# leaner-forever/SEGS-SLAM

Hardware: AMD Instinct MI355X
Metric: mapper train-iters/sec (fwd+bwd raster) (higher is better)
Workload: dtype f32; 1 GPU; 1080p_3m: 3000000 Gaussians, 1920x1080, 1 keyframe per GPU, fwd+bwd raster; P=3000000, P_visible=2096178, num_rendered=10472370, instances_binned=7913347, instances_live=6766534, width=1920, height=1080, parallelism=keyframe-dp1, forward=resident (no host sync), hipgraph=off

## Files before the change

segs-slam_amd/csrc/binning.hip:

```cpp
#include <hip/hip_runtime.h>
#include <cstdint>
#include "gs_layout.h"
#include "kernels.h"

namespace segs {

constexpr int PREFIX_ROWS = PREFIX_ROWS_PER_WG;

__global__ void __launch_bounds__(1024) scan_block_sums_kernel(uint32_t* __restrict__ block_sums, int nblocks,
                                                               const uint32_t* __restrict__ depth_range,
                                                               uint32_t* __restrict__ total) {
  __shared__ uint32_t w_sum[16], w_dmax[16], w_dnmin[16];
  const int tid = threadIdx.x, lane = tid & 63, wv = tid >> 6;
  uint32_t sum = 0, dmax = 0, dnmin = 0;
  for (int i = tid; i < nblocks; i += 1024) {
    sum += block_sums[i];
    dmax = max(dmax, depth_range[i]);
    dnmin = max(dnmin, depth_range[nblocks + i]);
  }
#pragma unroll
  for (int off = 32; off > 0; off >>= 1) {
    sum += __shfl_down(sum, off, 64);
    dmax = max(dmax, (uint32_t)__shfl_down((int)dmax, off, 64));
    dnmin = max(dnmin, (uint32_t)__shfl_down((int)dnmin, off, 64));
// ... 200 lines not shown
  const uint64_t kc = km.dbits < 0 ? (key >> 32) : (((key >> 32) << km.dbits) | (uint64_t)((uint32_t)key - km.dmin));
  return (uint32_t)(kc >> shift) & ((1u << BITS) - 1u);
}
template <int BITS>
__device__ __forceinline__ uint32_t digit_of(uint32_t key, int shift, KeyMap km) { return ((key - km.dmin) >> shift) & ((1u << BITS) - 1u); }

template <int BITS>
__device__ __forceinline__ uint64_t match_digit(uint32_t d, uint64_t valid, int nbits) {
  uint64_t peers = valid;
#pragma unroll
  for (int bit = 0; bit < BITS; bit++) {
    if (bit < nbits) {
      const bool set = (d >> bit) & 1u;
      const uint64_t m = __ballot(set);
      peers &= set ? m : ~m;
    }
  }
  return peers;
}
__device__ __forceinline__ uint32_t mbcnt(uint64_t m) {
  return __builtin_amdgcn_mbcnt_hi((uint32_t)(m >> 32), __builtin_amdgcn_mbcnt_lo((uint32_t)m, 0u));
}

template <typename K, int BITS>
__global__ void __launch_bounds__(SORT_THREADS) radix_count_kernel(const K* __restrict__ keys, int n, int shift,
                                                                    uint32_t dmin, int dbits,
                                                                    uint32_t* __restrict__ tile_prefix, uint32_t* __restrict__ chunk_hist,
                                                                    int nblocks, int nchunks,
                                                                    const uint32_t* __restrict__ n_dev, int drop_dead, int chunk_tiles,
                                                                    int nbits ) {
  const KeyMap km{dmin, dbits};
  if (n_dev) n = (int)min(*n_dev, (uint32_t)n);
  constexpr int NDIG = 1 << BITS;
  constexpr int DPT = NDIG / SORT_THREADS;
  __shared__ uint32_t cnt[4][NDIG];
  const int tid = threadIdx.x, lane = tid & 63, wv = tid >> 6;
  const uint32_t dmask = (1u << nbits) - 1u;
  uint32_t* my = cnt[wv];
  uint32_t running[DPT];
#pragma unroll
  for (int j = 0; j < DPT; j++) running[j] = 0u;
  K kreg[SORT_ITEMS_PER_THREAD], knext[SORT_ITEMS_PER_THREAD];
  const int chunks_in_use = (int)(((size_t)n + (size_t)SORT_TILE * chunk_tiles - 1) / ((size_t)SORT_TILE * chunk_tiles));
  const int chunks_per_xcd = (chunks_in_use + 7) >> 3;
  const int chunk_id = (int)(blockIdx.x & 7u) * chunks_per_xcd + (int)(blockIdx.x >> 3);
  if ((int)(blockIdx.x >> 3) >= chunks_per_xcd) {
    const int col = 8 * chunks_per_xcd + ((int)(blockIdx.x >> 3) - chunks_per_xcd) * 8 + (int)(blockIdx.x & 7u);
    if (col < nchunks) {
      constexpr int ND = 1 << BITS;
      for (int d = threadIdx.x; d < ND; d += SORT_THREADS) chunk_hist[(size_t)d * nchunks + col] = 0u;
    }
    return;
  }
  if (chunk_id >= nchunks) return;
  const int b0 = chunk_id * chunk_tiles;
  auto load_tile = [&](int b, K* dst) {
    const size_t wave_base = (size_t)b * SORT_TILE + (size_t)wv * (SORT_TILE / 4);
#pragma unroll
    for (int r = 0; r < SORT_ITEMS_PER_THREAD; r++) {
      const size_t i = wave_base + (size_t)r * 64 + lane;
      dst[r] = (b < nblocks && i < (size_t)n) ? keys[i] : (K)DEAD_KEY_OF(K);
    }
  };
  load_tile(b0, kreg);
  for (int t = 0; t < chunk_tiles; t++) {
    const int b = b0 + t;
    if (b >= nblocks) break;
    for (int i = tid; i < 4 * NDIG; i += SORT_THREADS) (&cnt[0][0])[i] = 0;
    if (t + 1 < chunk_tiles) load_tile(b + 1, knext);
    __syncthreads();
    const size_t wave_base = (size_t)b * SORT_TILE + (size_t)wv * (SORT_TILE / 4);
#pragma unroll
    for (int r = 0; r < SORT_ITEMS_PER_THREAD; r++) {
      const size_t i = wave_base + (size_t)r * 64 + lane;
      if (i < (size_t)n && !(drop_dead && kreg[r] == (K)DEAD_KEY_OF(K))) atomicAdd(&my[digit_of<BITS>(kreg[r], shift, km) & dmask], 1u);
    }
    __syncthreads();
#pragma unroll
    for (int j = 0; j < DPT; j++) {
      const int d = tid * DPT + j;
      tile_prefix[(size_t)b * NDIG + d] = running[j];
      running[j] += cnt[0][d] + cnt[1][d] + cnt[2][d] + cnt[3][d];
    }
    __syncthreads();
#pragma unroll
    for (int r = 0; r < SORT_ITEMS_PER_THREAD; r++) kreg[r] = knext[r];
  }
#pragma unroll
  for (int j = 0; j < DPT; j++) chunk_hist[(size_t)(tid * DPT + j) * nchunks + chunk_id] = running[j];
}

__global__ void __launch_bounds__(256) radix_scan_kernel(uint32_t* __restrict__ block_hist, int nblocks,
                                                         uint32_t* __restrict__ digit_totals) {
  constexpr int ITEMS = 8;
  __shared__ uint32_t wave_tot[4];
  const int tid = threadIdx.x, lane = tid & 63, wv = tid >> 6;
  uint32_t* row = block_hist + (size_t)blockIdx.x * nblocks;
  uint32_t carry = 0;
  for (int base = 0; base < nblocks; base += 256 * ITEMS) {
    const int i0 = base + tid * ITEMS;
    uint32_t v[ITEMS], sum = 0;
#pragma unroll
    for (int q = 0; q < ITEMS; q++) { v[q] = (i0 + q < nblocks) ? row[i0 + q] : 0u; sum += v[q]; }
    uint32_t x = sum;
#pragma unroll
    for (int off = 1; off < 64; off <<= 1) {
      const uint32_t y = __shfl_up(x, off, 64);
      if (lane >= off) x += y;
    }
    if (lane == 63) wave_tot[wv] = x;
    __syncthreads();
    uint32_t wbase = 0, total = 0;
#pragma unroll
    for (int w = 0; w < 4; w++) { const uint32_t t = wave_tot[w]; if (w < wv) wbase += t; total += t; }
    uint32_t run = carry + wbase + x - sum;
#pragma unroll
    for (int q = 0; q < ITEMS; q++) { if (i0 + q < nblocks) row[i0 + q] = run; run += v[q]; }
    carry += total;
    __syncthreads();
  }
  if (tid == 0) digit_totals[blockIdx.x] = carry;
}

template <typename K, int BITS, bool AUX>
__global__ void __launch_bounds__(SORT_THREADS) radix_scatter_kernel(
    const K* __restrict__ keys_in, const uint32_t* __restrict__ vals_in, K* __restrict__ keys_out,
    uint32_t* __restrict__ vals_out, int n, int shift, uint32_t dmin, int dbits, const uint32_t* __restrict__ tile_prefix,
    const uint32_t* __restrict__ chunk_prefix , const uint32_t* __restrict__ digit_totals,
    int nblocks, int nchunks, const uint32_t* __restrict__ n_dev, int drop_dead, uint32_t* __restrict__ n_live_out,
    const uint32_t* __restrict__ aux_in, uint32_t* __restrict__ aux_out, int nbits ,
    int chunk_tiles ,
    int pack_shift ,
    uint2* __restrict__ ranges_out ,
    uint32_t* __restrict__ status, uint32_t* __restrict__ status_mirror ,
    int write_keys ) {
  const KeyMap km{dmin, dbits};
  const uint32_t dmask = (1u << nbits) - 1u;
  if (ranges_out != nullptr && status != nullptr && blockIdx.x == 0 && threadIdx.x == 0) {
    const uint32_t ntot = status[0];
    const uint32_t over = (ntot > (uint32_t)n || status[2] != 0u) ? 1u : 0u;
    status[2] = 0u;
    status[3] = over;
    const uint32_t live = min(n_dev ? *n_dev : ntot, min(ntot, (uint32_t)n));
    status[1] = live;
    if (status_mirror) { status_mirror[0] = ntot; status_mirror[1] = live; status_mirror[3] = over; }
  }
  if (n_dev) n = (int)min(*n_dev, (uint32_t)n);
  constexpr int NDIG = 1 << BITS;
  constexpr int DPT = NDIG / SORT_THREADS;
  static_assert(NDIG % SORT_THREADS == 0 && BITS <= 11, "digit | rank << BITS must fit the rank of 2048 keys");
  __shared__ K s_keys[SORT_TILE];
  __shared__ uint32_t s_vals[SORT_TILE];
  __shared__ uint32_t s_aux[AUX ? SORT_TILE : 1];
  __shared__ uint32_t cnt[4][NDIG];
  __shared__ uint32_t local_start[NDIG];
  __shared__ int32_t gdelta[NDIG];
  __shared__ uint32_t scan_tmp[4];
  const int tid = threadIdx.x, lane = tid & 63, wv = tid >> 6;
  for (int i = tid; i < 4 * NDIG; i += SORT_THREADS) (&cnt[0][0])[i] = 0;
  __syncthreads();

#if defined(SEGS_MEASURE) && defined(SORT_TILE_IDENTITY)
  const int tile_id = (int)blockIdx.x;
#else
  const int tiles_in_use = (int)(((size_t)n + SORT_TILE - 1) / SORT_TILE);
  const int tiles_per_xcd = (tiles_in_use + 7) >> 3;
  const int tile_id = (int)(blockIdx.x & 7u) * tiles_per_xcd + (int)(blockIdx.x >> 3);
  if (tiles_in_use == 0 && n_live_out != nullptr && blockIdx.x == 0 && tid == 0) *n_live_out = 0u;
  if ((int)(blockIdx.x >> 3) >= tiles_per_xcd) return;
#endif
  if (tile_id >= nblocks) return;
  const size_t tile_base = (size_t)tile_id * SORT_TILE;
  const size_t wave_base = tile_base + (size_t)wv * (SORT_TILE / 4);
  const int nvalid = (size_t)n > tile_base ? (int)min((size_t)SORT_TILE, (size_t)n - tile_base) : 0;

  K key[SORT_ITEMS_PER_THREAD];
  uint32_t val[SORT_ITEMS_PER_THREAD];
  uint32_t aux[AUX ? SORT_ITEMS_PER_THREAD : 1];
  uint32_t drank[SORT_ITEMS_PER_THREAD];
  volatile uint32_t* my = cnt[wv];
#pragma unroll
  for (int r = 0; r < SORT_ITEMS_PER_THREAD; r++) {
    const size_t i = wave_base + (size_t)r * 64 + lane;
    const bool valid = i < (size_t)n;
    key[r] = valid ? keys_in[i] : (K)0;
    val[r] = vals_in ? (valid ? vals_in[i] : 0u) : (uint32_t)i;
    if (AUX) aux[r] = valid ? aux_in[val[r]] : 0u;
    if (!AUX && pack_shift > 0 && valid) val[r] |= min(aux_in[i], (0xFFFFFFFFu >> pack_shift)) << pack_shift;
  }
#pragma unroll
  for (int r = 0; r < SORT_ITEMS_PER_THREAD; r++) {
    const size_t i = wave_base + (size_t)r * 64 + lane;
    const bool valid = i < (size_t)n && !(drop_dead && key[r] == (K)DEAD_KEY_OF(K));
    const uint32_t d = valid ? (digit_of<BITS>(key[r], shift, km) & dmask) : 0u;
    const uint64_t vmask = __ballot(valid);
    const uint64_t peers = match_digit<BITS>(d, vmask, nbits);
    const uint32_t below = mbcnt(peers);
    uint32_t old = 0;
    if (valid) old = my[d];
    __builtin_amdgcn_wave_barrier();
    if (valid && below == 0) my[d] = old + (uint32_t)__popcll(peers);
    __builtin_amdgcn_wave_barrier();
    drank[r] = valid ? (d | ((old + below) << BITS)) : 0xFFFFFFFFu;
  }
  __syncthreads();

  uint32_t run[DPT], tot[DPT], thread_run = 0, thread_tot = 0;
#pragma unroll
  for (int j = 0; j < DPT; j++) {
    const int d = tid * DPT + j;
    uint32_t r = 0;
#pragma unroll
    for (int w = 0; w < 4; w++) { const uint32_t c = cnt[w][d]; cnt[w][d] = r; r += c; }
    run[j] = r; thread_run += r;
// ... 11 lines not shown
  for (int off = 1; off < 64; off <<= 1) {
    uint32_t y = __shfl_up(tx, off, 64);
    if (lane >= off) tx += y;
  }
  __shared__ uint32_t tot_tmp[4];
  if (lane == 63) tot_tmp[wv] = tx;
  __syncthreads();
  uint32_t lbase = 0, gbase = 0;
  for (int w = 0; w < wv; w++) { lbase += scan_tmp[w]; gbase += tot_tmp[w]; }
  uint32_t lstart = lbase + x - thread_run, gstart = gbase + tx - thread_tot;
#pragma unroll
  for (int j = 0; j < DPT; j++) {
    const int d = tid * DPT + j;
    local_start[d] = lstart;
    gdelta[d] = (int32_t)(gstart + chunk_prefix[(size_t)d * nchunks + tile_id / chunk_tiles] +
                          tile_prefix[(size_t)tile_id * NDIG + d] - lstart);
    lstart += run[j]; gstart += tot[j];
  }
  const int nout = drop_dead ? (int)(scan_tmp[0] + scan_tmp[1] + scan_tmp[2] + scan_tmp[3]) : nvalid;
  if (n_live_out != nullptr && tile_id == 0 && tid == 0) *n_live_out = tot_tmp[0] + tot_tmp[1] + tot_tmp[2] + tot_tmp[3];
  __syncthreads();

#pragma unroll
  for (int r = 0; r < SORT_ITEMS_PER_THREAD; r++) {
    if (drank[r] != 0xFFFFFFFFu) {
      const uint32_t d = drank[r] & (uint32_t)(NDIG - 1);
      const uint32_t pos = local_start[d] + cnt[wv][d] + (drank[r] >> BITS);
      s_keys[pos] = key[r];
      s_vals[pos] = val[r];
      if (AUX) s_aux[pos] = aux[r];
    }
  }
  __syncthreads();
#pragma unroll 4
  for (int r = 0; r < SORT_ITEMS_PER_THREAD; r++) {
    const int lp = r * SORT_THREADS + tid;
    if (lp < nout) {
      const K k = s_keys[lp];
#if defined(SEGS_MEASURE) && defined(ABLATE_SCATTER_LINEAR)
      const size_t gp = tile_base + (size_t)lp + (size_t)(gdelta[digit_of<BITS>(k, shift, km) & dmask] & 0);
#else
      const size_t gp = (size_t)((int64_t)lp + (int64_t)gdelta[digit_of<BITS>(k, shift, km) & dmask]);
#endif
#if defined(SEGS_MEASURE) && defined(ABLATE_SCATTER_NO_STORE)
      if (k == (K)0x12345677 && gp == 77) keys_out[gp] = k;
      continue;
#endif
      if (write_keys) keys_out[gp] = k;
      vals_out[gp] = s_vals[lp];
      if (AUX) aux_out[gp] = s_aux[lp];
      if constexpr (sizeof(K) == 4) {
        if (ranges_out != nullptr) {
          const K prev = lp > 0 ? s_keys[lp - 1] : ~k, next = lp + 1 < nout ? s_keys[lp + 1] : ~k;
          if (k != prev) atomicMin(&ranges_out[k].x, (uint32_t)gp);
          if (k != next) atomicMax(&ranges_out[k].y, (uint32_t)gp + 1u);
        }
      }
    }
  }
}

#define SEGS_INSTANTIATE_RADIX(K, BITS)                                                                                          \
  template __global__ void radix_count_kernel<K, BITS>(const K*, int, int, uint32_t, int, uint32_t*, uint32_t*, int, int,       \
                                                       const uint32_t*, int, int, int);                                                  \
  template __global__ void radix_scatter_kernel<K, BITS, false>(const K*, const uint32_t*, K*, uint32_t*, int, int, uint32_t, int, \
                                                                const uint32_t*, const uint32_t*, const uint32_t*, int, int,        \
                                                                const uint32_t*, int, uint32_t*, const uint32_t*, uint32_t*, int, int, int, \
                                                                uint2*, uint32_t*, uint32_t*, int);
SEGS_INSTANTIATE_RADIX(uint64_t, 8)
SEGS_INSTANTIATE_RADIX(uint32_t, 8)
SEGS_INSTANTIATE_RADIX(uint32_t, 9)
SEGS_INSTANTIATE_RADIX(uint32_t, 11)
#undef SEGS_INSTANTIATE_RADIX
#define SEGS_INSTANTIATE_AUX(BITS)                                                                                                     \
  template __global__ void radix_scatter_kernel<uint32_t, BITS, true>(const uint32_t*, const uint32_t*, uint32_t*, uint32_t*, int, int, \
                                                                      uint32_t, int, const uint32_t*, const uint32_t*, const uint32_t*, \
                                                                      int, int, const uint32_t*, int, uint32_t*, const uint32_t*, uint32_t*, int, int, int, \
                                                                      uint2*, uint32_t*, uint32_t*, int);
SEGS_INSTANTIATE_AUX(8)
SEGS_INSTANTIATE_AUX(9)
#undef SEGS_INSTANTIATE_AUX

__global__ void __launch_bounds__(256) identify_tile_ranges_kernel(int L, const uint32_t* __restrict__ keys,
                                                                   uint2* __restrict__ ranges, const uint32_t* __restrict__ n_dev,
                                                                   uint32_t* __restrict__ status, uint32_t* __restrict__ status_mirror,
                                                                   const uint32_t* __restrict__ n_live ) {
  static_assert(RANGE_KEYS_PER_THREAD == 4, "one uint4 per thread");
  const int idx = blockIdx.x * 256 + threadIdx.x;
  if (n_dev) {
    const uint32_t n = *n_dev;
    if (idx == 0 && status) {
      const uint32_t over = (n > (uint32_t)L || status[2] != 0u) ? 1u : 0u;
      status[2] = 0u;
      status[3] = over;
      const uint32_t live = n_live ? min(*n_live, min(n, (uint32_t)L)) : min(n, (uint32_t)L);
      status[1] = live;
      if (status_mirror) { status_mirror[0] = n; status_mirror[1] = live; status_mirror[3] = over; }
    }
    L = (int)min(n, (uint32_t)L);
  }
  if (n_live) L = (int)min(*n_live, (uint32_t)L);
  const int i0 = idx * RANGE_KEYS_PER_THREAD;
  if (i0 >= L) return;
// ... 132 lines not shown
```

segs-slam_amd/csrc/capi.hip:

```cpp
#include <hip/hip_runtime.h>
#include <cstdio>
#include <cstdlib>
#include <algorithm>
#include <cstring>
#include <string>
#include <vector>
#include "../../include/segs_raster.h"
#include "gs_layout.h"
#include "kernels.h"

using namespace segs;

namespace {
thread_local std::string g_err;
}
int segs::set_error(int code, const char* what) {
  g_err = what;
  return code;
}
int segs::set_hip_error(hipError_t e, const char* where) {
  g_err = std::string(where) + ": " + hipGetErrorString(e);
  return (int)e > 0 ? (int)e : 1;
}

// ... 48 lines not shown
uint32_t getHigherMsb(uint32_t n) {
  uint32_t msb = sizeof(n) * 4, step = msb;
  while (step > 1) {
    step /= 2;
    if (n >> msb) msb += step; else msb -= step;
  }
  if (n >> msb) msb++;
  return msb;
}

int count_chunk_tiles(int nblocks) {
#ifdef SEGS_MEASURE
  static const int chunk_override = [] { const char* e = getenv("SEGS_COUNT_CHUNK"); const int v = e ? atoi(e) : 0; return (v == 1 || v == 2 || v == 4) ? v : 0; }();
  if (chunk_override > 0) return chunk_override;
#endif
  return nblocks <= 256 ? 1 : (nblocks <= 2048 ? 2 : SORT_COUNT_CHUNK_TILES);
}
struct SortFusion {
  uint2* ranges = nullptr;
  uint32_t* status = nullptr;
  uint32_t* status_mirror = nullptr;
  bool keep_sorted_keys = true;
};
template <typename K, int BITS = 8>
int sort_pairs(char* bin, const BinningLayout& L, int n, int end_bit, uint32_t dmin, int dbits, hipStream_t st,
               const uint32_t* n_dev = nullptr, bool drop_dead = false, bool iota_vals = false, const uint32_t* aux_in = nullptr,
               uint32_t* aux_final = nullptr, int pack_shift = 0 ,
               const SortFusion& fuse = SortFusion(), const K* first_keys = nullptr ) {
  if (n <= 0) return SEGS_OK;
  uint32_t* n_live = (uint32_t*)(bin + L.n_live);
  const int passes = (end_bit + BITS - 1) / BITS;
  int side = passes & 1;
  uint32_t* tile_prefix = (uint32_t*)(bin + L.tile_prefix);
  uint32_t* chunk_hist = (uint32_t*)(bin + L.chunk_hist);
  uint32_t* digit_totals = (uint32_t*)(bin + L.digit_totals);
  const int chunk_tiles = count_chunk_tiles(L.nblocks);
  const int nchunks = (L.nblocks + chunk_tiles - 1) / chunk_tiles;
  for (int p = 0; p < passes; p++) {
    const K* kin = (p == 0 && first_keys) ? first_keys : (const K*)(bin + L.keys[side]);
    const uint32_t* vin = (const uint32_t*)(bin + L.vals[side]);
    K* kout = (K*)(bin + L.keys[side ^ 1]);
    uint32_t* vout = (uint32_t*)(bin + L.vals[side ^ 1]);
    const int shift = BITS * p;
    const int drop = drop_dead && p == 0;
    const uint32_t* n_in = (drop_dead && p > 0) ? n_live : n_dev;
    const int nbits = std::min(BITS, end_bit - shift);
    { PROF(K_RADIX_COUNT);
    radix_count_kernel<K, BITS><<<(nchunks + 7) / 8 * 8, SORT_THREADS, 0, st>>>(kin, n, shift, dmin, dbits, tile_prefix, chunk_hist, L.nblocks, nchunks, n_in, drop, chunk_tiles, nbits);
    }
    LAUNCH_TRY("radix_count_kernel");
    const bool last = p == passes - 1;
    uint2* fr = last ? fuse.ranges : nullptr;
    uint32_t* fs = last ? fuse.status : nullptr;
    uint32_t* fm = last ? fuse.status_mirror : nullptr;
    const int wk = (last && !fuse.keep_sorted_keys) ? 0 : 1;
    { PROF(K_RADIX_SCAN);
    radix_scan_kernel<<<1 << BITS, 256, 0, st>>>(chunk_hist, nchunks, digit_totals);
    }
    LAUNCH_TRY("radix_scan_kernel");
    if (iota_vals && p == 0) vin = nullptr;
    const int scatter_grid = (L.nblocks + 7) / 8 * 8;
    { PROF(K_RADIX_SCATTER);
    if constexpr (sizeof(K) == 4) {
      if (aux_in && aux_final && p == passes - 1) {
        radix_scatter_kernel<K, BITS, true><<<scatter_grid, SORT_THREADS, 0, st>>>(kin, vin, kout, vout, n, shift, dmin, dbits, tile_prefix, chunk_hist,
                                                                        digit_totals, L.nblocks, nchunks, n_in, drop,
                                                                        drop ? n_live : nullptr, aux_in, aux_final, nbits, chunk_tiles, 0, fr, fs, fm, wk);
      } else {
        radix_scatter_kernel<K, BITS, false><<<scatter_grid, SORT_THREADS, 0, st>>>(kin, vin, kout, vout, n, shift, dmin, dbits, tile_prefix, chunk_hist,
                                                                         digit_totals, L.nblocks, nchunks, n_in, drop,
                                                                         drop ? n_live : nullptr, (pack_shift > 0 && p == 0) ? aux_in : nullptr, nullptr,
                                                                         nbits, chunk_tiles, (p == 0) ? pack_shift : 0, fr, fs, fm, wk);
      }
    } else {
      radix_scatter_kernel<K, BITS, false><<<scatter_grid, SORT_THREADS, 0, st>>>(kin, vin, kout, vout, n, shift, dmin, dbits, tile_prefix, chunk_hist,
                                                                       digit_totals, L.nblocks, nchunks, n_in, drop,
                                                                       drop ? n_live : nullptr, nullptr, nullptr, nbits, chunk_tiles, 0, nullptr, nullptr, nullptr, 1);
    }
    }
    LAUNCH_TRY("radix_scatter_kernel");
    side ^= 1;
  }
  return SEGS_OK;
}

struct Geom {
  GeomLayout L;
  char* base;
  float* rec() const { return (float*)(base + L.rec); }
  BinInfo* bin() const { return (BinInfo*)(base + L.bin); }
  uint32_t* offsets() const { return (uint32_t*)(base + L.offsets); }
  int* radii_internal() const { return (int*)(base + L.radii_internal); }
  uint32_t* block_sums() const { return (uint32_t*)(base + L.block_sums); }
  uint32_t* num_rendered() const { return (uint32_t*)(base + L.num_rendered); }
  uint32_t* clamped() const { return (uint32_t*)(base + L.clamped); }
  float* gacc() const { return (float*)(base + L.gacc); }
  uint32_t* touched() const { return (uint32_t*)(base + L.touched); }
};
Geom geom_at(char* p, int P) { return Geom{geom_layout(P), align_ptr(p)}; }
Geom geom_at(char* p, int P, int rows) {
  Geom g{geom_layout(rows), align_ptr(p)};
  g.L.P = P;
  g.L.nblocks = (P + 255) / 256;
  return g;
}

// ... 15 lines not shown
  LAUNCH_TRY("preprocess_fwd_kernel");
  return SEGS_OK;
}

int run_binning(const Geom& G, char* bin, const BinningLayout& BL, const GaussSortLayout& GS, uint2* ranges, int P, int n_cap,
                const uint32_t* n_dev, uint32_t dmin, int dbits, uint32_t dcull, uint32_t gx, uint32_t gy, uint32_t* total_out,
                hipStream_t st, bool depth_keys_ready = false, bool drop_dead = false, bool nine_bit_depth = false,
                const uint32_t* depth_keys_src = nullptr ) {
  const int bit = (int)getHigherMsb(gx * gy);
  char* gbin = bin + GS.base;
  const BinningLayout& GL = GS.inner;
  const int gside = (nine_bit_depth ? (dbits + 8) / 9 : (dbits + 7) / 8) & 1;
  if (!depth_keys_ready) { PROF(K_DUPLICATE);
  make_depth_keys_kernel<<<G.L.nblocks, 256, 0, st>>>(P, G.bin(), dcull, (uint32_t*)(gbin + GL.keys[gside]), (uint32_t*)(gbin + GL.vals[gside]),
                                                      ranges, (int)(gx * gy));
  }
  LAUNCH_TRY("make_depth_keys_kernel");
  const bool drop_culled = depth_keys_ready;
  int idx_bits = 1;
  while (idx_bits < 32 && ((uint64_t)1 << idx_bits) < (uint64_t)P) idx_bits++;
  int pack_shift = (32 - idx_bits >= 6 && !(g_flags & SEGS_RASTER_GATHER_TILES_TOUCHED)) ? idx_bits : 0;
  if (pack_shift && (g_flags & SEGS_RASTER_TEST_NARROW_PACK)) pack_shift = 30;
  uint32_t* aux_final = pack_shift ? nullptr : G.offsets();
  int rc = nine_bit_depth ? sort_pairs<uint32_t, 9>(gbin, GL, P, dbits, dmin, dbits, st, nullptr, drop_culled, true, G.touched(), aux_final, pack_shift, SortFusion(), depth_keys_src)
                          : sort_pairs<uint32_t>(gbin, GL, P, dbits, dmin, dbits, st, nullptr, drop_culled, true, G.touched(), aux_final, pack_shift, SortFusion(), depth_keys_src);
  if (rc) return rc;
  uint32_t* order = (uint32_t*)(gbin + GL.vals[0]);
  const uint32_t* ng_dev = drop_culled ? (const uint32_t*)(gbin + GL.n_live) : nullptr;
  uint32_t* sums2 = (uint32_t*)(bin + GS.block_sums);
  uint32_t* first_owner = (uint32_t*)(bin + GS.first_owner);
  const int prefix_wgs = (P + 256 * PREFIX_ROWS_PER_WG - 1) / (256 * PREFIX_ROWS_PER_WG);
  { PROF(K_SCAN);
  ordered_block_sums_kernel<<<prefix_wgs, 256, 0, st>>>(P, pack_shift ? G.touched() : G.offsets(), nullptr, sums2, G.offsets(), ng_dev, order, pack_shift);
  }
  LAUNCH_TRY("ordered_block_sums_kernel");
#ifdef SEGS_MEASURE
  static const bool no_wide = getenv("SEGS_NO_WIDE_DIGIT") != nullptr;
#else
  constexpr bool no_wide = false;
#endif
  const bool wide_digit = !no_wide && bit <= 11 && BL.nblocks <= SORT_WIDE_MAX_TILES;
  const int tpasses = wide_digit ? 1 : (bit + 7) / 8;
  const int side = tpasses & 1;
  { PROF(K_SCAN);
  ordered_offsets_kernel<<<prefix_wgs, 256, 0, st>>>(P, sums2, G.offsets(), total_out, ng_dev, first_owner,
                                                      (uint32_t)(n_cap / EMIT_SLOTS_PER_WG + 2));
  }
  LAUNCH_TRY("ordered_offsets_kernel");
  const bool unfused = (g_flags & SEGS_RASTER_UNFUSED_BINNING) != 0u;
  { PROF(K_DUPLICATE);
  duplicate_with_keys_kernel<<<(n_cap + EMIT_SLOTS_PER_WG - 1) / EMIT_SLOTS_PER_WG, 256, 0, st>>>(P, n_cap, G.rec(), order, G.offsets(),
                                                                    (uint32_t*)(bin + BL.keys[side]), (uint32_t*)(bin + BL.vals[side]), gx, n_dev,
                                                                    drop_dead ? 1 : 0, ng_dev, first_owner);
  }
  LAUNCH_TRY("duplicate_with_keys_kernel");
  SortFusion fuse;
  const bool fused_ranges = !unfused && tpasses >= 2;
  if (fused_ranges) {
    fuse.ranges = ranges;
    fuse.status = n_dev ? total_out : nullptr;
    fuse.status_mirror = n_dev ? g_status_mirror : nullptr;
    fuse.keep_sorted_keys = n_dev == nullptr;
  }
  rc = wide_digit ? sort_pairs<uint32_t, 11>(bin, BL, n_cap, bit, 0u, 0, st, n_dev, drop_dead, false, nullptr, nullptr, 0, fuse)
// ... 698 lines not shown
```

segs-slam_amd/csrc/gs_layout.h:

```cpp
#pragma once
#include <algorithm>
#include <cstddef>
#include <cstdint>

namespace segs {

constexpr int TILE_X = 16;
constexpr int TILE_Y = 16;
constexpr int NUM_CHANNELS = 3;

constexpr float LOG2E = 1.4426950408889634f;

constexpr int REC_DWORDS = 16;
enum RecField { REC_X = 0, REC_Y, REC_A2, REC_B2, REC_C2, REC_O, REC_R, REC_G, REC_B, REC_DEPTH, REC_RECT_MIN, REC_RECT_MAX, REC_CA, REC_CB, REC_CC };

struct BinInfo { uint32_t depth_bits, rect_min, rect_max, tiles_touched; };
constexpr uint32_t ID_BITS = 28;
constexpr uint32_t ID_MASK = (1u << ID_BITS) - 1u;
constexpr int MAX_GAUSSIANS = 1 << ID_BITS;

constexpr int GACC_DWORDS = 16;

constexpr size_t ALIGN = 256;
inline size_t align_up(size_t v, size_t a = ALIGN) { return (v + a - 1) / a * a; }
// ... 14 lines not shown
  g.block_sums = o;     o = align_up(o + (size_t)(g.nblocks + 1) * 4 * 3);
  g.clamped = o;        o = align_up(o + (size_t)P * 4);
  g.num_rendered = o;   o = align_up(o + 64);
  g.gacc = o;           o = align_up(o + (size_t)P * GACC_DWORDS * 4);
  g.touched = o;        o = align_up(o + (size_t)P * 4);
  g.total = o + ALIGN;
  return g;
}

struct ImageLayout {
  size_t ranges, final_T, n_contrib, total;
};
inline ImageLayout image_layout(int W, int H) {
  ImageLayout l{};
  const size_t tiles = (size_t)((W + TILE_X - 1) / TILE_X) * ((H + TILE_Y - 1) / TILE_Y);
  size_t o = 0;
  l.ranges = o;    o = align_up(o + tiles * 8);
  l.final_T = o;   o = align_up(o + (size_t)W * H * 4);
  l.n_contrib = o; o = align_up(o + (size_t)W * H * 4);
  l.total = o + ALIGN;
  return l;
}

#ifndef SEGS_SORT_ITEMS_PER_THREAD
#define SEGS_SORT_ITEMS_PER_THREAD 8
#endif
constexpr int SORT_ITEMS_PER_THREAD = SEGS_SORT_ITEMS_PER_THREAD;
constexpr int SORT_THREADS = 256;
constexpr int SORT_TILE = SORT_ITEMS_PER_THREAD * SORT_THREADS;
constexpr int PREFIX_ROWS_PER_WG = 8;
constexpr int EMIT_SLOTS_PER_WG = 512;
constexpr int SORT_COUNT_CHUNK_TILES = 4;
constexpr int RANGE_KEYS_PER_THREAD = 4;
constexpr int SORT_WIDE_DIGITS = 2048;
constexpr int SORT_WIDE_MAX_TILES = 1024;
constexpr int SORT_MAX_DIGITS = 512;

struct BinningLayout {
  size_t keys[2], vals[2], tile_prefix, chunk_hist, digit_totals, n_live, total;
  int nchunks;
  int R, nblocks;
};
inline BinningLayout binning_layout(int R) {
  BinningLayout b{};
  b.R = R;
  b.nblocks = (R + SORT_TILE - 1) / SORT_TILE;
  size_t o = 0;
  for (int i = 0; i < 2; i++) { b.keys[i] = o; o = align_up(o + (size_t)R * 8); }
  for (int i = 0; i < 2; i++) { b.vals[i] = o; o = align_up(o + (size_t)R * 4); }
  b.nchunks = b.nblocks;
  const size_t cols = (size_t)(b.nblocks > 0 ? b.nblocks : 1);
  const size_t matrix = std::max((size_t)SORT_MAX_DIGITS * cols, (size_t)SORT_WIDE_DIGITS * std::min(cols, (size_t)SORT_WIDE_MAX_TILES));
  b.tile_prefix = o;  o = align_up(o + matrix * 4);
  b.chunk_hist = o;   o = align_up(o + matrix * 4);
  b.digit_totals = o; o = align_up(o + SORT_WIDE_DIGITS * 4);
  b.n_live = o;       o = align_up(o + 4);
  b.total = o + ALIGN;
  return b;
}
struct GaussSortLayout {
  size_t base, block_sums, first_owner, total;
  BinningLayout inner;
};
inline GaussSortLayout gauss_sort_layout(int R, int P) {
  GaussSortLayout g{};
  g.inner = binning_layout(P);
  g.base = align_up(binning_layout(R).total);
  g.block_sums = g.base + align_up(g.inner.total);
  g.first_owner = g.block_sums + align_up((size_t)((P + 255) / 256 + 4) * 4);
  g.total = g.first_owner + align_up((size_t)(R / EMIT_SLOTS_PER_WG + 4) * 4) + ALIGN;
  return g;
}

inline char* align_ptr(char* p) { return (char*)(((uintptr_t)p + ALIGN - 1) / ALIGN * ALIGN); }
inline const char* align_ptr(const char* p) { return (const char*)(((uintptr_t)p + ALIGN - 1) / ALIGN * ALIGN); }
// ... 3 lines not shown
```

segs-slam_amd/csrc/kernels.h:

```cpp
#pragma once
#include <hip/hip_runtime.h>
#include <cstdint>
#include "gs_layout.h"

namespace segs {

int set_error(int code, const char* what);
int set_hip_error(hipError_t e, const char* where);


__global__ void preprocess_fwd_kernel(
    int P, const float* __restrict__ means3D, const float* __restrict__ scales, float mod,
    const float* __restrict__ rotations, const float* __restrict__ opacities, const float* __restrict__ colors,
    const float* __restrict__ cov3D_precomp, const float* __restrict__ viewmatrix, const float* __restrict__ projmatrix,
    int W, int H, float tan_fovx, float tan_fovy, float focal_x, float focal_y, uint32_t gx, uint32_t gy,
    int* __restrict__ radii, float* __restrict__ rec, BinInfo* __restrict__ bin, uint32_t* __restrict__ block_sums,
    uint32_t* __restrict__ depth_range, const float* __restrict__ shs, int D, int M, const float* __restrict__ cam_pos,
    uint32_t* __restrict__ clamped, uint32_t flags, uint32_t* __restrict__ depth_keys, uint32_t* __restrict__ depth_vals,
    uint2* __restrict__ ranges, int num_tiles, uint32_t* __restrict__ depth_overflow, uint32_t* __restrict__ touched_dense);
constexpr uint32_t DEPTH_KEY_MIN = 0x3E4CCCCDu;
constexpr int DEPTH_KEY_BITS = 27;

__global__ void visible_filter_kernel(
    int P, const float* __restrict__ means3D, const float* __restrict__ scales, float mod,
// ... 17 lines not shown
    float* __restrict__ dL_dcov3D, float* __restrict__ dL_dscale, float* __restrict__ dL_drot, int clean_gacc,
    const float* __restrict__ dz_in, float* __restrict__ cam_partials);
__global__ void camera_grad_reduce_kernel(const float* __restrict__ partials, int nblocks, float* __restrict__ dL_dview,
                                          float* __restrict__ dL_dproj);
__global__ void sh_backward_kernel(int P, const float* __restrict__ means3D, const int* __restrict__ radii,
                                   const float* __restrict__ shs, int D, int M, const float* __restrict__ cam_pos,
                                   const uint32_t* __restrict__ clamped, const float* __restrict__ dL_dcolor,
                                   float* __restrict__ dL_dmean3D, float* __restrict__ dL_dsh);

__global__ void scan_block_sums_kernel(uint32_t* __restrict__ block_sums, int nblocks, const uint32_t* __restrict__ depth_range,
                                       uint32_t* __restrict__ total);
__global__ void ordered_offsets_kernel(int P, const uint32_t* __restrict__ block_sums, uint32_t* __restrict__ incl,
                                       uint32_t* __restrict__ total_out, const uint32_t* __restrict__ ng_dev,
                                       uint32_t* __restrict__ first_owner, uint32_t owner_entries);
__global__ void duplicate_with_keys_kernel(int P, int R, const float* __restrict__ rec,
                                           const uint32_t* __restrict__ order, const uint32_t* __restrict__ incl,
                                           uint32_t* __restrict__ keys, uint32_t* __restrict__ vals, uint32_t gx,
                                           const uint32_t* __restrict__ n_dev, int mark_dead, const uint32_t* __restrict__ ng_dev,
                                           const uint32_t* __restrict__ first_owner);
constexpr uint32_t RANGE_EMPTY_START = 0xFFFFFFFFu;
__global__ void normalize_ranges_kernel(int num_tiles, uint2* __restrict__ ranges);
constexpr uint32_t PREPROCESS_TIGHT_RECT = 0x80000000u;
constexpr uint32_t DEAD_KEY = 0xFFFFFFFFu;
template <typename K, int BITS>
__global__ void radix_count_kernel(const K* __restrict__ keys, int n, int shift, uint32_t dmin, int dbits,
                                   uint32_t* __restrict__ tile_prefix, uint32_t* __restrict__ chunk_hist, int nblocks, int nchunks,
                                   const uint32_t* __restrict__ n_dev, int drop_dead, int chunk_tiles, int nbits);
__global__ void radix_scan_kernel(uint32_t* __restrict__ block_hist, int nblocks, uint32_t* __restrict__ digit_totals);
template <typename K, int BITS, bool AUX>
__global__ void radix_scatter_kernel(const K* __restrict__ keys_in, const uint32_t* __restrict__ vals_in,
                                     K* __restrict__ keys_out, uint32_t* __restrict__ vals_out, int n, int shift,
                                     uint32_t dmin, int dbits, const uint32_t* __restrict__ tile_prefix, const uint32_t* __restrict__ chunk_prefix,
                                     const uint32_t* __restrict__ digit_totals, int nblocks, int nchunks,
                                     const uint32_t* __restrict__ n_dev, int drop_dead, uint32_t* __restrict__ n_live_out,
                                     const uint32_t* __restrict__ aux_in, uint32_t* __restrict__ aux_out, int nbits, int chunk_tiles, int pack_shift,
                                     uint2* __restrict__ ranges_out, uint32_t* __restrict__ status, uint32_t* __restrict__ status_mirror,
                                     int write_keys);
__global__ void identify_tile_ranges_kernel(int L, const uint32_t* __restrict__ keys, uint2* __restrict__ ranges,
                                            const uint32_t* __restrict__ n_dev, uint32_t* __restrict__ status,
                                            uint32_t* __restrict__ status_mirror, const uint32_t* __restrict__ n_live);

__global__ void render_fwd_kernel(const uint2* __restrict__ ranges, const uint32_t* __restrict__ point_list, int W, int H,
                                  const float* __restrict__ rec, const float* __restrict__ bg,
                                  float* __restrict__ final_T, uint32_t* __restrict__ n_contrib, float* __restrict__ out_color);
__global__ void render_bwd_kernel(const uint2* __restrict__ ranges, const uint32_t* __restrict__ point_list, int W, int H,
                                  const float* __restrict__ rec, const float* __restrict__ bg,
                                  const float* __restrict__ final_T, const uint32_t* __restrict__ n_contrib,
                                  const float* __restrict__ dL_dpix, float* __restrict__ gacc, uint32_t num_tiles);
__global__ void render_bwd_mfma_kernel(const uint2* __restrict__ ranges, const uint32_t* __restrict__ point_list, int W, int H,
                                       const float* __restrict__ rec, const float* __restrict__ bg,
                                       const float* __restrict__ final_T, const uint32_t* __restrict__ n_contrib,
                                       const float* __restrict__ dL_dpix, float* __restrict__ gacc, uint32_t num_tiles);
// ... 27 lines not shown
```

Before: 1007 iters/s.

## Template radix sort on tile size and alias scatter LDS staging buffers

```diff
diff --git a/segs-slam_amd/csrc/binning.hip b/segs-slam_amd/csrc/binning.hip
--- a/segs-slam_amd/csrc/binning.hip
+++ b/segs-slam_amd/csrc/binning.hip
@@ -246,7 +246,7 @@
   return __builtin_amdgcn_mbcnt_hi((uint32_t)(m >> 32), __builtin_amdgcn_mbcnt_lo((uint32_t)m, 0u));
 }
 
-template <typename K, int BITS>
+template <typename K, int BITS, int TILE>
 __global__ void __launch_bounds__(SORT_THREADS) radix_count_kernel(const K* __restrict__ keys, int n, int shift,
                                                                     uint32_t dmin, int dbits,
                                                                     uint32_t* __restrict__ tile_prefix, uint32_t* __restrict__ chunk_hist,
@@ -257,6 +257,8 @@
   if (n_dev) n = (int)min(*n_dev, (uint32_t)n);
   constexpr int NDIG = 1 << BITS;
   constexpr int DPT = NDIG / SORT_THREADS;
+  constexpr int ITEMS = TILE / SORT_THREADS;
+  static_assert(TILE % SORT_THREADS == 0 && ITEMS >= 1, "whole rows of 64 keys per wave");
   __shared__ uint32_t cnt[4][NDIG];
   const int tid = threadIdx.x, lane = tid & 63, wv = tid >> 6;
   const uint32_t dmask = (1u << nbits) - 1u;
@@ -264,8 +266,8 @@
   uint32_t running[DPT];
 #pragma unroll
   for (int j = 0; j < DPT; j++) running[j] = 0u;
-  K kreg[SORT_ITEMS_PER_THREAD], knext[SORT_ITEMS_PER_THREAD];
-  const int chunks_in_use = (int)(((size_t)n + (size_t)SORT_TILE * chunk_tiles - 1) / ((size_t)SORT_TILE * chunk_tiles));
+  K kreg[ITEMS], knext[ITEMS];
+  const int chunks_in_use = (int)(((size_t)n + (size_t)TILE * chunk_tiles - 1) / ((size_t)TILE * chunk_tiles));
   const int chunks_per_xcd = (chunks_in_use + 7) >> 3;
   const int chunk_id = (int)(blockIdx.x & 7u) * chunks_per_xcd + (int)(blockIdx.x >> 3);
   if ((int)(blockIdx.x >> 3) >= chunks_per_xcd) {
@@ -279,9 +281,9 @@
   if (chunk_id >= nchunks) return;
   const int b0 = chunk_id * chunk_tiles;
   auto load_tile = [&](int b, K* dst) {
-    const size_t wave_base = (size_t)b * SORT_TILE + (size_t)wv * (SORT_TILE / 4);
-#pragma unroll
-    for (int r = 0; r < SORT_ITEMS_PER_THREAD; r++) {
+    const size_t wave_base = (size_t)b * TILE + (size_t)wv * (TILE / 4);
+#pragma unroll
+    for (int r = 0; r < ITEMS; r++) {
       const size_t i = wave_base + (size_t)r * 64 + lane;
       dst[r] = (b < nblocks && i < (size_t)n) ? keys[i] : (K)DEAD_KEY_OF(K);
     }
@@ -293,9 +295,9 @@
     for (int i = tid; i < 4 * NDIG; i += SORT_THREADS) (&cnt[0][0])[i] = 0;
     if (t + 1 < chunk_tiles) load_tile(b + 1, knext);
     __syncthreads();
-    const size_t wave_base = (size_t)b * SORT_TILE + (size_t)wv * (SORT_TILE / 4);
-#pragma unroll
-    for (int r = 0; r < SORT_ITEMS_PER_THREAD; r++) {
+    const size_t wave_base = (size_t)b * TILE + (size_t)wv * (TILE / 4);
+#pragma unroll
+    for (int r = 0; r < ITEMS; r++) {
       const size_t i = wave_base + (size_t)r * 64 + lane;
       if (i < (size_t)n && !(drop_dead && kreg[r] == (K)DEAD_KEY_OF(K))) atomicAdd(&my[digit_of<BITS>(kreg[r], shift, km) & dmask], 1u);
     }
@@ -308,7 +310,7 @@
     }
     __syncthreads();
 #pragma unroll
-    for (int r = 0; r < SORT_ITEMS_PER_THREAD; r++) kreg[r] = knext[r];
+    for (int r = 0; r < ITEMS; r++) kreg[r] = knext[r];
   }
 #pragma unroll
   for (int j = 0; j < DPT; j++) chunk_hist[(size_t)(tid * DPT + j) * nchunks + chunk_id] = running[j];
@@ -346,7 +348,7 @@
   if (tid == 0) digit_totals[blockIdx.x] = carry;
 }
 
-template <typename K, int BITS, bool AUX>
+template <typename K, int BITS, bool AUX, int TILE>
 __global__ void __launch_bounds__(SORT_THREADS) radix_scatter_kernel(
     const K* __restrict__ keys_in, const uint32_t* __restrict__ vals_in, K* __restrict__ keys_out,
     uint32_t* __restrict__ vals_out, int n, int shift, uint32_t dmin, int dbits, const uint32_t* __restrict__ tile_prefix,
@@ -372,12 +374,17 @@
   if (n_dev) n = (int)min(*n_dev, (uint32_t)n);
   constexpr int NDIG = 1 << BITS;
   constexpr int DPT = NDIG / SORT_THREADS;
-  static_assert(NDIG % SORT_THREADS == 0 && BITS <= 11, "digit | rank << BITS must fit the rank of 2048 keys");
-  __shared__ K s_keys[SORT_TILE];
-  __shared__ uint32_t s_vals[SORT_TILE];
-  __shared__ uint32_t s_aux[AUX ? SORT_TILE : 1];
-  __shared__ uint32_t cnt[4][NDIG];
-  __shared__ uint32_t local_start[NDIG];
+  constexpr int ITEMS = TILE / SORT_THREADS;
+  static_assert(NDIG % SORT_THREADS == 0 && BITS <= 11 && TILE <= 4096, "digit | rank << BITS must fit the rank of a tile's keys");
+  static_assert(TILE % SORT_THREADS == 0 && ITEMS >= 1, "whole rows of 64 keys per wave");
+  constexpr size_t RANK_BYTES = (size_t)5 * NDIG * 4;
+  constexpr size_t STAGE_BYTES = (size_t)TILE * (sizeof(K) + 4 + (AUX ? 4 : 0));
+  __shared__ __attribute__((aligned(16))) unsigned char lds_shared[RANK_BYTES > STAGE_BYTES ? RANK_BYTES : STAGE_BYTES];
+  uint32_t (*cnt)[NDIG] = reinterpret_cast<uint32_t (*)[NDIG]>(lds_shared);
+  uint32_t* const local_start = reinterpret_cast<uint32_t*>(lds_shared) + 4 * NDIG;
+  K* const s_keys = reinterpret_cast<K*>(lds_shared);
+  uint32_t* const s_vals = reinterpret_cast<uint32_t*>(lds_shared + (size_t)TILE * sizeof(K));
+  uint32_t* const s_aux = s_vals + TILE;
   __shared__ int32_t gdelta[NDIG];
   __shared__ uint32_t scan_tmp[4];
   const int tid = threadIdx.x, lane = tid & 63, wv = tid >> 6;
@@ -387,24 +394,24 @@
 #if defined(SEGS_MEASURE) && defined(SORT_TILE_IDENTITY)
   const int tile_id = (int)blockIdx.x;
 #else
-  const int tiles_in_use = (int)(((size_t)n + SORT_TILE - 1) / SORT_TILE);
+  const int tiles_in_use = (int)(((size_t)n + TILE - 1) / TILE);
   const int tiles_per_xcd = (tiles_in_use + 7) >> 3;
   const int tile_id = (int)(blockIdx.x & 7u) * tiles_per_xcd + (int)(blockIdx.x >> 3);
   if (tiles_in_use == 0 && n_live_out != nullptr && blockIdx.x == 0 && tid == 0) *n_live_out = 0u;
   if ((int)(blockIdx.x >> 3) >= tiles_per_xcd) return;
 #endif
   if (tile_id >= nblocks) return;
-  const size_t tile_base = (size_t)tile_id * SORT_TILE;
-  const size_t wave_base = tile_base + (size_t)wv * (SORT_TILE / 4);
-  const int nvalid = (size_t)n > tile_base ? (int)min((size_t)SORT_TILE, (size_t)n - tile_base) : 0;
-
-  K key[SORT_ITEMS_PER_THREAD];
-  uint32_t val[SORT_ITEMS_PER_THREAD];
-  uint32_t aux[AUX ? SORT_ITEMS_PER_THREAD : 1];
-  uint32_t drank[SORT_ITEMS_PER_THREAD];
+  const size_t tile_base = (size_t)tile_id * TILE;
+  const size_t wave_base = tile_base + (size_t)wv * (TILE / 4);
+  const int nvalid = (size_t)n > tile_base ? (int)min((size_t)TILE, (size_t)n - tile_base) : 0;
+
+  K key[ITEMS];
+  uint32_t val[ITEMS];
+  uint32_t aux[AUX ? ITEMS : 1];
+  uint32_t drank[ITEMS];
   volatile uint32_t* my = cnt[wv];
 #pragma unroll
-  for (int r = 0; r < SORT_ITEMS_PER_THREAD; r++) {
+  for (int r = 0; r < ITEMS; r++) {
     const size_t i = wave_base + (size_t)r * 64 + lane;
     const bool valid = i < (size_t)n;
     key[r] = valid ? keys_in[i] : (K)0;
@@ -413,7 +420,7 @@
     if (!AUX && pack_shift > 0 && valid) val[r] |= min(aux_in[i], (0xFFFFFFFFu >> pack_shift)) << pack_shift;
   }
 #pragma unroll
-  for (int r = 0; r < SORT_ITEMS_PER_THREAD; r++) {
+  for (int r = 0; r < ITEMS; r++) {
     const size_t i = wave_base + (size_t)r * 64 + lane;
     const bool valid = i < (size_t)n && !(drop_dead && key[r] == (K)DEAD_KEY_OF(K));
     const uint32_t d = valid ? (digit_of<BITS>(key[r], shift, km) & dmask) : 0u;
@@ -471,10 +478,17 @@
   __syncthreads();
 
 #pragma unroll
-  for (int r = 0; r < SORT_ITEMS_PER_THREAD; r++) {
+  for (int r = 0; r < ITEMS; r++) {
     if (drank[r] != 0xFFFFFFFFu) {
       const uint32_t d = drank[r] & (uint32_t)(NDIG - 1);
-      const uint32_t pos = local_start[d] + cnt[wv][d] + (drank[r] >> BITS);
+      drank[r] = local_start[d] + cnt[wv][d] + (drank[r] >> BITS);
+    }
+  }
+  __syncthreads();
+#pragma unroll
+  for (int r = 0; r < ITEMS; r++) {
+    if (drank[r] != 0xFFFFFFFFu) {
+      const uint32_t pos = drank[r];
       s_keys[pos] = key[r];
       s_vals[pos] = val[r];
       if (AUX) s_aux[pos] = aux[r];
@@ -482,7 +496,7 @@
   }
   __syncthreads();
 #pragma unroll 4
-  for (int r = 0; r < SORT_ITEMS_PER_THREAD; r++) {
+  for (int r = 0; r < ITEMS; r++) {
     const int lp = r * SORT_THREADS + tid;
     if (lp < nout) {
       const K k = s_keys[lp];
@@ -509,25 +523,35 @@
   }
 }
 
-#define SEGS_INSTANTIATE_RADIX(K, BITS)                                                                                          \
-  template __global__ void radix_count_kernel<K, BITS>(const K*, int, int, uint32_t, int, uint32_t*, uint32_t*, int, int,       \
-                                                       const uint32_t*, int, int, int);                                                  \
-  template __global__ void radix_scatter_kernel<K, BITS, false>(const K*, const uint32_t*, K*, uint32_t*, int, int, uint32_t, int, \
+#define SEGS_INSTANTIATE_RADIX(K, BITS, TILE)                                                                                    \
+  template __global__ void radix_count_kernel<K, BITS, TILE>(const K*, int, int, uint32_t, int, uint32_t*, uint32_t*, int, int, \
+                                                             const uint32_t*, int, int, int);                                            \
+  template __global__ void radix_scatter_kernel<K, BITS, false, TILE>(const K*, const uint32_t*, K*, uint32_t*, int, int, uint32_t, int, \
                                                                 const uint32_t*, const uint32_t*, const uint32_t*, int, int,        \
                                                                 const uint32_t*, int, uint32_t*, const uint32_t*, uint32_t*, int, int, int, \
                                                                 uint2*, uint32_t*, uint32_t*, int);
-SEGS_INSTANTIATE_RADIX(uint64_t, 8)
-SEGS_INSTANTIATE_RADIX(uint32_t, 8)
-SEGS_INSTANTIATE_RADIX(uint32_t, 9)
-SEGS_INSTANTIATE_RADIX(uint32_t, 11)
-#undef SEGS_INSTANTIATE_RADIX
-#define SEGS_INSTANTIATE_AUX(BITS)                                                                                                     \
-  template __global__ void radix_scatter_kernel<uint32_t, BITS, true>(const uint32_t*, const uint32_t*, uint32_t*, uint32_t*, int, int, \
+#define SEGS_INSTANTIATE_AUX(BITS, TILE)                                                                                                     \
+  template __global__ void radix_scatter_kernel<uint32_t, BITS, true, TILE>(const uint32_t*, const uint32_t*, uint32_t*, uint32_t*, int, int, \
                                                                       uint32_t, int, const uint32_t*, const uint32_t*, const uint32_t*, \
                                                                       int, int, const uint32_t*, int, uint32_t*, const uint32_t*, uint32_t*, int, int, int, \
                                                                       uint2*, uint32_t*, uint32_t*, int);
-SEGS_INSTANTIATE_AUX(8)
-SEGS_INSTANTIATE_AUX(9)
+#define SEGS_INSTANTIATE_TILE(TILE)      \
+  SEGS_INSTANTIATE_RADIX(uint64_t, 8, TILE) \
+  SEGS_INSTANTIATE_RADIX(uint32_t, 8, TILE) \
+  SEGS_INSTANTIATE_RADIX(uint32_t, 9, TILE) \
+  SEGS_INSTANTIATE_RADIX(uint32_t, 11, TILE) \
+  SEGS_INSTANTIATE_AUX(8, TILE)             \
+  SEGS_INSTANTIATE_AUX(9, TILE)
+SEGS_INSTANTIATE_TILE(2048)
+#ifdef SEGS_MEASURE
+SEGS_INSTANTIATE_TILE(1024)
+SEGS_INSTANTIATE_TILE(512)
+#else
+SEGS_INSTANTIATE_RADIX(uint32_t, 9, 1024)
+SEGS_INSTANTIATE_AUX(9, 1024)
+#endif
+#undef SEGS_INSTANTIATE_TILE
+#undef SEGS_INSTANTIATE_RADIX
 #undef SEGS_INSTANTIATE_AUX
 
 __global__ void __launch_bounds__(256) identify_tile_ranges_kernel(int L, const uint32_t* __restrict__ keys,
diff --git a/segs-slam_amd/csrc/capi.hip b/segs-slam_amd/csrc/capi.hip
--- a/segs-slam_amd/csrc/capi.hip
+++ b/segs-slam_amd/csrc/capi.hip
@@ -94,20 +94,30 @@
   uint32_t* status_mirror = nullptr;
   bool keep_sorted_keys = true;
 };
-template <typename K, int BITS = 8>
-int sort_pairs(char* bin, const BinningLayout& L, int n, int end_bit, uint32_t dmin, int dbits, hipStream_t st,
-               const uint32_t* n_dev = nullptr, bool drop_dead = false, bool iota_vals = false, const uint32_t* aux_in = nullptr,
-               uint32_t* aux_final = nullptr, int pack_shift = 0 ,
-               const SortFusion& fuse = SortFusion(), const K* first_keys = nullptr ) {
-  if (n <= 0) return SEGS_OK;
+int sort_tile_choice(size_t n, int bits) {
+#ifdef SEGS_MEASURE
+  static const int forced[3] = {[] { const char* e = getenv("SEGS_SORT_TILE_B8"); return e ? atoi(e) : 0; }(),
+                                [] { const char* e = getenv("SEGS_SORT_TILE_B9"); return e ? atoi(e) : 0; }(),
+                                [] { const char* e = getenv("SEGS_SORT_TILE_B11"); return e ? atoi(e) : 0; }()};
+  const int f = forced[bits == 8 ? 0 : (bits == 9 ? 1 : 2)];
+  if (f == 512 || f == 1024 || f == 2048) return f;
+#endif
+  return sort_tile_keys(n, bits);
+}
+template <typename K, int BITS, int TILE>
+int sort_pairs_tiled(char* bin, const BinningLayout& L, int n, int end_bit, uint32_t dmin, int dbits, hipStream_t st,
+                     const uint32_t* n_dev, bool drop_dead, bool iota_vals, const uint32_t* aux_in, uint32_t* aux_final, int pack_shift,
+                     const SortFusion& fuse, const K* first_keys) {
   uint32_t* n_live = (uint32_t*)(bin + L.n_live);
   const int passes = (end_bit + BITS - 1) / BITS;
   int side = passes & 1;
   uint32_t* tile_prefix = (uint32_t*)(bin + L.tile_prefix);
   uint32_t* chunk_hist = (uint32_t*)(bin + L.chunk_hist);
   uint32_t* digit_totals = (uint32_t*)(bin + L.digit_totals);
-  const int chunk_tiles = count_chunk_tiles(L.nblocks);
-  const int nchunks = (L.nblocks + chunk_tiles - 1) / chunk_tiles;
+  const int nblocks = sort_tile_count((size_t)n, TILE);
+  if (nblocks > L.nblocks) return fail(SEGS_ERR_INVALID_ARGUMENT, "sort scratch holds too few count-matrix columns for this tile");
+  const int chunk_tiles = count_chunk_tiles(nblocks);
+  const int nchunks = (nblocks + chunk_tiles - 1) / chunk_tiles;
   for (int p = 0; p < passes; p++) {
     const K* kin = (p == 0 && first_keys) ? first_keys : (const K*)(bin + L.keys[side]);
     const uint32_t* vin = (const uint32_t*)(bin + L.vals[side]);
@@ -118,7 +128,7 @@
     const uint32_t* n_in = (drop_dead && p > 0) ? n_live : n_dev;
     const int nbits = std::min(BITS, end_bit - shift);
     { PROF(K_RADIX_COUNT);
-    radix_count_kernel<K, BITS><<<(nchunks + 7) / 8 * 8, SORT_THREADS, 0, st>>>(kin, n, shift, dmin, dbits, tile_prefix, chunk_hist, L.nblocks, nchunks, n_in, drop, chunk_tiles, nbits);
+    radix_count_kernel<K, BITS, TILE><<<(nchunks + 7) / 8 * 8, SORT_THREADS, 0, st>>>(kin, n, shift, dmin, dbits, tile_prefix, chunk_hist, nblocks, nchunks, n_in, drop, chunk_tiles, nbits);
     }
     LAUNCH_TRY("radix_count_kernel");
     const bool last = p == passes - 1;
@@ -131,22 +141,26 @@
     }
     LAUNCH_TRY("radix_scan_kernel");
     if (iota_vals && p == 0) vin = nullptr;
-    const int scatter_grid = (L.nblocks + 7) / 8 * 8;
+    const int scatter_grid = (nblocks + 7) / 8 * 8;
     { PROF(K_RADIX_SCATTER);
-    if constexpr (sizeof(K) == 4) {
+    if constexpr (sizeof(K) == 4 && BITS != 11) {
       if (aux_in && aux_final && p == passes - 1) {
-        radix_scatter_kernel<K, BITS, true><<<scatter_grid, SORT_THREADS, 0, st>>>(kin, vin, kout, vout, n, shift, dmin, dbits, tile_prefix, chunk_hist,
-                                                                        digit_totals, L.nblocks, nchunks, n_in, drop,
+        radix_scatter_kernel<K, BITS, true, TILE><<<scatter_grid, SORT_THREADS, 0, st>>>(kin, vin, kout, vout, n, shift, dmin, dbits, tile_prefix, chunk_hist,
+                                                                        digit_totals, nblocks, nchunks, n_in, drop,
                                                                         drop ? n_live : nullptr, aux_in, aux_final, nbits, chunk_tiles, 0, fr, fs, fm, wk);
       } else {
-        radix_scatter_kernel<K, BITS, false><<<scatter_grid, SORT_THREADS, 0, st>>>(kin, vin, kout, vout, n, shift, dmin, dbits, tile_prefix, chunk_hist,
-                                                                         digit_totals, L.nblocks, nchunks, n_in, drop,
+        radix_scatter_kernel<K, BITS, false, TILE><<<scatter_grid, SORT_THREADS, 0, st>>>(kin, vin, kout, vout, n, shift, dmin, dbits, tile_prefix, chunk_hist,
+                                                                         digit_totals, nblocks, nchunks, n_in, drop,
                                                                          drop ? n_live : nullptr, (pack_shift > 0 && p == 0) ? aux_in : nullptr, nullptr,
                                                                          nbits, chunk_tiles, (p == 0) ? pack_shift : 0, fr, fs, fm, wk);
       }
+    } else if constexpr (sizeof(K) == 4) {
+      radix_scatter_kernel<K, BITS, false, TILE><<<scatter_grid, SORT_THREADS, 0, st>>>(kin, vin, kout, vout, n, shift, dmin, dbits, tile_prefix, chunk_hist,
+                                                                       digit_totals, nblocks, nchunks, n_in, drop,
+                                                                       drop ? n_live : nullptr, nullptr, nullptr, nbits, chunk_tiles, 0, fr, fs, fm, wk);
     } else {
-      radix_scatter_kernel<K, BITS, false><<<scatter_grid, SORT_THREADS, 0, st>>>(kin, vin, kout, vout, n, shift, dmin, dbits, tile_prefix, chunk_hist,
-                                                                       digit_totals, L.nblocks, nchunks, n_in, drop,
+      radix_scatter_kernel<K, BITS, false, TILE><<<scatter_grid, SORT_THREADS, 0, st>>>(kin, vin, kout, vout, n, shift, dmin, dbits, tile_prefix, chunk_hist,
+                                                                       digit_totals, nblocks, nchunks, n_in, drop,
                                                                        drop ? n_live : nullptr, nullptr, nullptr, nbits, chunk_tiles, 0, nullptr, nullptr, nullptr, 1);
     }
     }
@@ -154,6 +168,26 @@
     side ^= 1;
   }
   return SEGS_OK;
+}
+template <typename K, int BITS = 8>
+int sort_pairs(char* bin, const BinningLayout& L, int n, int end_bit, uint32_t dmin, int dbits, hipStream_t st,
+               const uint32_t* n_dev = nullptr, bool drop_dead = false, bool iota_vals = false, const uint32_t* aux_in = nullptr,
+               uint32_t* aux_final = nullptr, int pack_shift = 0 ,
+               const SortFusion& fuse = SortFusion(), const K* first_keys = nullptr ) {
+  if (n <= 0) return SEGS_OK;
+  switch (sort_tile_choice((size_t)n, BITS)) {
+#define SEGS_SORT_CASE(TILE) \
+    case TILE: return sort_pairs_tiled<K, BITS, TILE>(bin, L, n, end_bit, dmin, dbits, st, n_dev, drop_dead, iota_vals, aux_in, aux_final, pack_shift, fuse, first_keys);
+    SEGS_SORT_CASE(2048)
+#ifdef SEGS_MEASURE
+    SEGS_SORT_CASE(1024)
+    SEGS_SORT_CASE(512)
+#else
+    case 1024: if constexpr (sizeof(K) == 4 && BITS == 9) return sort_pairs_tiled<K, BITS, 1024>(bin, L, n, end_bit, dmin, dbits, st, n_dev, drop_dead, iota_vals, aux_in, aux_final, pack_shift, fuse, first_keys); break;
+#endif
+#undef SEGS_SORT_CASE
+  }
+  return fail(SEGS_ERR_INVALID_ARGUMENT, "sort tile not built");
 }
 
 struct Geom {
@@ -215,8 +249,10 @@
   int pack_shift = (32 - idx_bits >= 6 && !(g_flags & SEGS_RASTER_GATHER_TILES_TOUCHED)) ? idx_bits : 0;
   if (pack_shift && (g_flags & SEGS_RASTER_TEST_NARROW_PACK)) pack_shift = 30;
   uint32_t* aux_final = pack_shift ? nullptr : G.offsets();
-  int rc = nine_bit_depth ? sort_pairs<uint32_t, 9>(gbin, GL, P, dbits, dmin, dbits, st, nullptr, drop_culled, true, G.touched(), aux_final, pack_shift, SortFusion(), depth_keys_src)
-                          : sort_pairs<uint32_t>(gbin, GL, P, dbits, dmin, dbits, st, nullptr, drop_culled, true, G.touched(), aux_final, pack_shift, SortFusion(), depth_keys_src);
+  SortFusion depth_fuse;
+  depth_fuse.keep_sorted_keys = false;
+  int rc = nine_bit_depth ? sort_pairs<uint32_t, 9>(gbin, GL, P, dbits, dmin, dbits, st, nullptr, drop_culled, true, G.touched(), aux_final, pack_shift, depth_fuse, depth_keys_src)
+                          : sort_pairs<uint32_t>(gbin, GL, P, dbits, dmin, dbits, st, nullptr, drop_culled, true, G.touched(), aux_final, pack_shift, depth_fuse, depth_keys_src);
   if (rc) return rc;
   uint32_t* order = (uint32_t*)(gbin + GL.vals[0]);
   const uint32_t* ng_dev = drop_culled ? (const uint32_t*)(gbin + GL.n_live) : nullptr;
@@ -232,7 +268,7 @@
 #else
   constexpr bool no_wide = false;
 #endif
-  const bool wide_digit = !no_wide && bit <= 11 && BL.nblocks <= SORT_WIDE_MAX_TILES;
+  const bool wide_digit = !no_wide && bit <= 11 && n_cap <= SORT_WIDE_MAX_KEYS;
   const int tpasses = wide_digit ? 1 : (bit + 7) / 8;
   const int side = tpasses & 1;
   { PROF(K_SCAN);
diff --git a/segs-slam_amd/csrc/gs_layout.h b/segs-slam_amd/csrc/gs_layout.h
--- a/segs-slam_amd/csrc/gs_layout.h
+++ b/segs-slam_amd/csrc/gs_layout.h
@@ -60,19 +60,36 @@
   return l;
 }
 
-#ifndef SEGS_SORT_ITEMS_PER_THREAD
-#define SEGS_SORT_ITEMS_PER_THREAD 8
-#endif
-constexpr int SORT_ITEMS_PER_THREAD = SEGS_SORT_ITEMS_PER_THREAD;
 constexpr int SORT_THREADS = 256;
-constexpr int SORT_TILE = SORT_ITEMS_PER_THREAD * SORT_THREADS;
 constexpr int PREFIX_ROWS_PER_WG = 8;
 constexpr int EMIT_SLOTS_PER_WG = 512;
 constexpr int SORT_COUNT_CHUNK_TILES = 4;
 constexpr int RANGE_KEYS_PER_THREAD = 4;
 constexpr int SORT_WIDE_DIGITS = 2048;
-constexpr int SORT_WIDE_MAX_TILES = 1024;
+constexpr int SORT_WIDE_MAX_KEYS = 1 << 21;
 constexpr int SORT_MAX_DIGITS = 512;
+
+constexpr int SORT_TILE_MIN = 512, SORT_TILE_MAX = 2048;
+constexpr size_t sort_tile_limit(int tile, int bits) {
+  if (tile >= SORT_TILE_MAX) return ~(size_t)0;
+  return (bits == 9 && tile == 1024) ? ((size_t)1 << 20) : 0;
+}
+constexpr int sort_tile_keys(size_t n, int bits) {
+  for (int tile = SORT_TILE_MIN; tile < SORT_TILE_MAX; tile *= 2)
+    if (n <= sort_tile_limit(tile, bits)) return tile;
+  return SORT_TILE_MAX;
+}
+inline int sort_tile_count(size_t n, int tile) { return (int)((n + (size_t)tile - 1) / (size_t)tile); }
+inline int sort_count_columns(size_t n) {
+#ifdef SEGS_MEASURE
+  return sort_tile_count(n, SORT_TILE_MIN);
+#else
+  int cols = 0;
+  for (int bits : {8, 9, 11})
+    for (int tile = SORT_TILE_MIN; tile <= SORT_TILE_MAX; tile *= 2) cols = std::max(cols, sort_tile_count(std::min(n, sort_tile_limit(tile, bits)), tile));
+  return cols;
+#endif
+}
 
 struct BinningLayout {
   size_t keys[2], vals[2], tile_prefix, chunk_hist, digit_totals, n_live, total;
@@ -82,13 +99,14 @@
 inline BinningLayout binning_layout(int R) {
   BinningLayout b{};
   b.R = R;
-  b.nblocks = (R + SORT_TILE - 1) / SORT_TILE;
+  b.nblocks = sort_count_columns((size_t)R);
   size_t o = 0;
   for (int i = 0; i < 2; i++) { b.keys[i] = o; o = align_up(o + (size_t)R * 8); }
   for (int i = 0; i < 2; i++) { b.vals[i] = o; o = align_up(o + (size_t)R * 4); }
   b.nchunks = b.nblocks;
   const size_t cols = (size_t)(b.nblocks > 0 ? b.nblocks : 1);
-  const size_t matrix = std::max((size_t)SORT_MAX_DIGITS * cols, (size_t)SORT_WIDE_DIGITS * std::min(cols, (size_t)SORT_WIDE_MAX_TILES));
+  const size_t wide_cols = std::min(cols, (size_t)sort_count_columns((size_t)SORT_WIDE_MAX_KEYS));
+  const size_t matrix = std::max((size_t)SORT_MAX_DIGITS * cols, (size_t)SORT_WIDE_DIGITS * wide_cols);
   b.tile_prefix = o;  o = align_up(o + matrix * 4);
   b.chunk_hist = o;   o = align_up(o + matrix * 4);
   b.digit_totals = o; o = align_up(o + SORT_WIDE_DIGITS * 4);
diff --git a/segs-slam_amd/csrc/kernels.h b/segs-slam_amd/csrc/kernels.h
--- a/segs-slam_amd/csrc/kernels.h
+++ b/segs-slam_amd/csrc/kernels.h
@@ -63,12 +63,12 @@
 __global__ void normalize_ranges_kernel(int num_tiles, uint2* __restrict__ ranges);
 constexpr uint32_t PREPROCESS_TIGHT_RECT = 0x80000000u;
 constexpr uint32_t DEAD_KEY = 0xFFFFFFFFu;
-template <typename K, int BITS>
+template <typename K, int BITS, int TILE>
 __global__ void radix_count_kernel(const K* __restrict__ keys, int n, int shift, uint32_t dmin, int dbits,
                                    uint32_t* __restrict__ tile_prefix, uint32_t* __restrict__ chunk_hist, int nblocks, int nchunks,
                                    const uint32_t* __restrict__ n_dev, int drop_dead, int chunk_tiles, int nbits);
 __global__ void radix_scan_kernel(uint32_t* __restrict__ block_hist, int nblocks, uint32_t* __restrict__ digit_totals);
-template <typename K, int BITS, bool AUX>
+template <typename K, int BITS, bool AUX, int TILE>
 __global__ void radix_scatter_kernel(const K* __restrict__ keys_in, const uint32_t* __restrict__ vals_in,
                                      K* __restrict__ keys_out, uint32_t* __restrict__ vals_out, int n, int shift,
                                      uint32_t dmin, int dbits, const uint32_t* __restrict__ tile_prefix, const uint32_t* __restrict__ chunk_prefix,
```

Result: no change. 1015 iters/s, median of 6 (+0.8%).
